# johannes-graeter/limo

Measured on NVIDIA H100. Metric: BA windows/s (30 KF, 3k LM, 40k obs), higher is better.
Workload: dtype f64

## Files before the change

### limo_b200/csrc/kba_api.cu

```cuda
#include <algorithm>
#include <atomic>
#include <chrono>
#include <cmath>
#include <cstdio>
#include <cstdlib>
#include <cstring>
#include <functional>
#include <memory>
#include <string>
#include <thread>
#include <vector>

#include <cuda_runtime.h>

#include "kba_b200.h"
#include "kba_kernels.h"

using namespace kba;

static thread_local std::string g_last_error;
static int fail(int code, const std::string& msg) {
    g_last_error = msg;
    return code;
}
// ... 707 lines not shown
    b->bd.nr_cap_max = p.nr_cap_max; b->bd.fused = p.fused; b->bd.p_split = p.p_split;
    b->bd.solve_tiled = p.solve_tiled; b->bd.solve_split = p.solve_split; b->bd.solve_banded = p.solve_banded;
}

static int batch_create(kba_handle* h, int32_t n_windows, const kba_window* w, const int* rows_of, Purpose purpose, kba_batch** out) {
    if (!h || !w || !out || n_windows <= 0) return fail(KBA_ERR_BAD_ARG, "bad argument to kba_batch_create");
    CU(cudaSetDevice(h->device));
    std::string why;
    for (int i = 0; i < n_windows; ++i) {
        const int rc = validate_window(&w[i], why);
        if (rc != KBA_OK) return fail(rc, "window " + std::to_string(i) + ": " + why);
        if (w[i].n_kf < 3 && !w[i].landmarks_fixed)
            return fail(KBA_ERR_NOT_ENOUGH_KF, "window " + std::to_string(i) + ": fewer than 3 keyframes");
    }
    kba_batch* b = new kba_batch();
    b->h = h;
    BatchDev& bd = b->bd;
    bd.n_win = n_windows;
    b->desc_h.resize(n_windows);
    std::vector<WinShape> shapes(n_windows);
    long long kf = 0, cam = 0, lm = 0, obs = 0, chunks = 0, soff = 0, gp = 0, groups = 0;
    for (int i = 0; i < n_windows; ++i) {
        WinDesc& d = b->desc_h[i];
        memset(&d, 0, sizeof d);
        d.n_kf = w[i].n_kf; d.n_cam = w[i].n_cam; d.n_lm = w[i].n_lm; d.n_obs = w[i].n_obs; d.n_gp = w[i].n_gp;
        d.kf_off = (int)kf; d.cam_off = (int)cam; d.lm_off = (int)lm; d.obs_off = (int)obs; d.gp_off = (int)gp;
        d.chunk_off = (int)chunks; d.n_chunks = (w[i].n_lm + 31) / 32;
        d.grp_off = (int)groups; d.n_groups = (w[i].n_lm + 7) / 8;
        groups += d.n_groups;
        d.scale_kf0 = w[i].scale_kf0; d.scale_kf1 = w[i].scale_kf1;
        d.scale_weight = w[i].scale_weight; d.scale_value = w[i].scale_value;
        WinShape& ws = shapes[i];
        ws.rows = rows_of ? rows_of[i] : reduced_rows(w[i].n_kf, w[i].n_gp > 0 || w[i].plane_reg_weight > 0);
        ws.free_rows = window_rows(w[i]);
        ws.n_chunks = d.n_chunks; ws.n_groups = d.n_groups; ws.n_lm = w[i].n_lm;
        d.nr_cap = nr_cap_of(ws.rows);
        d.plane_reg_weight = w[i].plane_reg_weight; d.plane_dist_fixed = w[i].plane_dist_fixed;
        d.s_off = soff;
        soff += (long long)d.nr_cap * d.nr_cap;
        kf += w[i].n_kf; cam += w[i].n_cam; lm += w[i].n_lm; obs += w[i].n_obs; chunks += d.n_chunks; gp += w[i].n_gp;
        bd.max_obs = std::max(bd.max_obs, w[i].n_obs); bd.max_lm = std::max(bd.max_lm, w[i].n_lm);
        bd.max_kf = std::max(bd.max_kf, w[i].n_kf); bd.max_gp = std::max(bd.max_gp, w[i].n_gp);
    }
    b->lc.knobs = read_knobs();
    b->lc.plan = make_plan(shapes.data(), n_windows, h->sm_count, b->lc.knobs, purpose);
    apply_plan(b);
    const int nr_cap_max = b->lc.plan.nr_cap_max;
    if (obs > 2000000000LL) { b->release(); delete b; return fail(KBA_ERR_CAPACITY, "batch exceeds 2^31 observations"); }
    if (nr_cap_max > kMaxReducedRows) {
        b->release();
        delete b;
        return fail(KBA_ERR_CAPACITY, "reduced system larger than 1344 rows (128 keyframes with ground-plane blocks)");
    }
    bd.tot_kf = kf; bd.tot_cam = cam; bd.tot_lm = lm; bd.tot_obs = obs; bd.tot_chunks = (int)chunks; bd.tot_gp = gp;
    bd.tot_groups = (int)groups;
    b->lc.sm_count = h->sm_count;
    bd.cost_parts = std::max((bd.max_obs + 255) / 256, (bd.max_obs / 16 + bd.max_lm / 32 + 4 + 7) / 8);
    bd.bs_parts = (bd.max_lm + 15) / 16;
    const bool hp = !b->lc.plan.device_pack;
    int bad = 0;
    bad |= b->desc.alloc(n_windows, true);
    bad |= b->pose0.alloc(7 * kf, true); bad |= b->plane0.alloc(4 * kf, true); bad |= b->kf_fixed.alloc(kf, true);
    bad |= b->cam.alloc(kCamStride * cam, true);
    bad |= b->lm0.alloc(3 * lm, hp); bad |= b->lm_weight.alloc(lm, hp); bad |= b->lm_ptr.alloc(lm + n_windows, hp);
    bad |= b->obs_kf.alloc(obs, hp); bad |= b->obs_cam.alloc(obs, hp); bad |= b->obs_lm.alloc(obs, hp);
    bad |= b->obs_u.alloc(obs, hp); bad |= b->obs_v.alloc(obs, hp); bad |= b->obs_d.alloc(obs, hp);
    bad |= b->kf_ptr.alloc(kf + n_windows, hp); bad |= b->pm_lm.alloc(obs, hp); bad |= b->pm_cam.alloc(obs, hp);
    bad |= b->pm_u.alloc(obs, hp); bad |= b->pm_v.alloc(obs, hp); bad |= b->pm_d.alloc(obs, hp);
    bad |= b->chunk_lm0.alloc(chunks, hp); bad |= b->chunk_lm1.alloc(chunks, hp);
    bad |= b->chunk_k0.alloc(chunks, hp); bad |= b->chunk_k1.alloc(chunks, hp);
    bad |= b->lm_orig.alloc(lm, hp); bad |= b->obs_rank.alloc(obs, hp);
    if (hp) bad |= b->obs_orig.alloc(obs, true);
    bad |= b->grp_k0.alloc(groups, hp); bad |= b->grp_k1.alloc(groups, hp);
    if (b->lc.plan.device_pack) {
        bad |= b->r_lm_ptr.alloc(lm + n_windows, true); bad |= b->r_obs_kf.alloc(obs, true); bad |= b->r_obs_cam.alloc(obs, true);
        bad |= b->r_obs_u.alloc(obs, true); bad |= b->r_obs_v.alloc(obs, true); bad |= b->r_obs_d.alloc(obs, true);
        bad |= b->r_lm_pos.alloc(3 * lm, true); bad |= b->r_lm_weight.alloc(lm, true); bad |= b->r_gp_lm.alloc(gp, true);
        bad |= b->lm_user.alloc(3 * lm, true); bad |= b->rej_user.alloc(lm, true);
        bad |= b->dev_alloc(&b->raw.lm_inv, lm);
    }
    bad |= b->dev_alloc(&bd.grp_t0, groups); bad |= b->dev_alloc(&bd.grp_t1, groups); bad |= b->dev_alloc(&bd.grp_rs, groups);
    bad |= b->dev_alloc(&bd.grp_tiles, groups);
    bad |= b->dev_alloc(&bd.lin_tile, (size_t)(obs / 16) + (size_t)(lm / 32) + 4 * (size_t)n_windows + 4);
#ifdef KBA_PROF
    bad |= b->dev_alloc(&bd.prof, 16);
    if (!bad) cudaMemset(bd.prof, 0, 16 * sizeof(unsigned long long));
#endif
    bad |= b->dev_alloc(&bd.rt[0], (size_t)kPoseStride * kf); bad |= b->dev_alloc(&bd.rt[1], (size_t)kPoseStride * kf);
    {
        bd.panel_cap = 0;
        bd.vpanel = nullptr;
        bad |= b->dev_alloc(&bd.chunk_poff, chunks); bad |= b->dev_alloc(&bd.chunk_rs, chunks);
    }
    bad |= b->dev_alloc(&bd.chunk_t0, chunks); bad |= b->dev_alloc(&bd.chunk_t1, chunks); bad |= b->dev_alloc(&bd.obs_row, obs);
    bad |= b->state.alloc(n_windows, true); bad |= b->log.alloc((size_t)n_windows * kIterLogCap, true); bad |= b->wsp.alloc(n_windows, true);
    for (int q = 0; q < 2; ++q) { bad |= b->pose_out[q].alloc(7 * kf, true); bad |= b->lm_out[q].alloc(3 * lm, hp); }
    bad |= b->lm_active.alloc(lm, hp); bad |= b->n_active.alloc(1, true); bad |= b->jac_obs.alloc(1, true);
    bad |= b->plane_out[0].alloc(4 * kf, true); bad |= b->plane_out[1].alloc(4 * kf, true);
    bad |= b->gp_lm.alloc(gp, hp); bad |= b->gp_kf.alloc(gp, true); bad |= b->gp_weight.alloc(gp, true); bad |= b->gp_of_lm.alloc(lm, hp); bad |= b->gp_shared.alloc(gp, hp);
    bad |= b->dev_alloc(&bd.gp_lin, 14 * gp); bad |= b->dev_alloc(&bd.vgp, 30 * gp);
    bad |= b->dev_alloc(&bd.gp_kfb, gp ? 65 * (size_t)kf : 0);
    bad |= b->dev_alloc(&bd.gp_cost_x, n_windows); bad |= b->dev_alloc(&bd.gp_cost_c, n_windows);
    bad |= b->dev_alloc(&bd.off_pose, kf); bad |= b->dev_alloc(&bd.off_dir, kf); bad |= b->dev_alloc(&bd.off_dist, kf);
    bad |= b->dev_alloc(&bd.bkf, 27 * kf);
    bad |= b->dev_alloc(&bd.scale_f, (size_t)n_windows * nr_cap_max); bad |= b->dev_alloc(&bd.lambda_f, (size_t)n_windows * nr_cap_max);
    bad |= b->dev_alloc(&bd.grad_f, (size_t)n_windows * nr_cap_max); bad |= b->dev_alloc(&bd.delta_f, (size_t)n_windows * nr_cap_max);
    bad |= b->dev_alloc(&bd.lm_scale, 3 * lm); bad |= b->dev_alloc(&bd.lm_linv, 6 * lm); bad |= b->dev_alloc(&bd.lm_z, 3 * lm);
    bad |= b->dev_alloc(&bd.lm_g, 3 * lm); bad |= b->dev_alloc(&bd.lm_lambda, 3 * lm); bad |= b->dev_alloc(&bd.trim_val, 3 * lm);
    bad |= b->dev_alloc(&bd.trim_reject, lm);
    bad |= b->dev_alloc(&bd.res, 3 * obs); bad |= b->dev_alloc(&bd.jp, 18 * obs);
    if (!bd.fused) bad |= b->dev_alloc(&bd.jl, 9 * obs);
    else { bad |= b->dev_alloc(&bd.vobs, 18 * obs); bad |= b->dev_alloc(&bd.lm_run, lm); }
    bad |= b->dev_alloc(&bd.cost_part_x, (size_t)n_windows * bd.cost_parts); bad |= b->dev_alloc(&bd.cost_part_c, (size_t)n_windows * bd.cost_parts);
    bad |= b->dev_alloc(&bd.bs_part, (size_t)n_windows * bd.bs_parts * 4);
    bad |= b->dev_alloc(&bd.sred, (size_t)soff * bd.p_split); bad |= b->dev_alloc(&bd.amat, (size_t)soff);
    bad |= b->dev_alloc(&bd.chol_w, (size_t)n_windows * 32 * 32); bad |= b->dev_alloc(&bd.chol_invd, (size_t)n_windows * nr_cap_max);
    if (bad) {
        const std::string msg = std::string("device/pinned allocation failed: ") + cudaGetErrorString(cudaGetLastError());
        b->release(); delete b;
        return fail(KBA_ERR_CUDA, msg);
    }
    bd.desc = b->desc.d; bd.state = b->state.d; bd.log = b->log.d; bd.wsp = b->wsp.d;
    bd.pose0 = b->pose0.d; bd.plane0 = b->plane0.d; bd.pose[0] = b->pose_out[0].d; bd.pose[1] = b->pose_out[1].d;
    bd.kf_fixed = b->kf_fixed.d; bd.cam = b->cam.d;
    bd.lm0 = b->lm0.d; bd.lm[0] = b->lm_out[0].d; bd.lm[1] = b->lm_out[1].d; bd.lm_weight = b->lm_weight.d;
    bd.lm_active = b->lm_active.d; bd.lm_ptr = b->lm_ptr.d;
    bd.obs_kf = b->obs_kf.d; bd.obs_cam = b->obs_cam.d; bd.obs_lm = b->obs_lm.d;
    bd.obs_u = b->obs_u.d; bd.obs_v = b->obs_v.d; bd.obs_d = b->obs_d.d;
    bd.kf_ptr = b->kf_ptr.d; bd.pm_lm = b->pm_lm.d; bd.pm_cam = b->pm_cam.d; bd.pm_u = b->pm_u.d; bd.pm_v = b->pm_v.d; bd.pm_d = b->pm_d.d;
    bd.chunk_lm0 = b->chunk_lm0.d; bd.chunk_lm1 = b->chunk_lm1.d; bd.chunk_k0 = b->chunk_k0.d; bd.chunk_k1 = b->chunk_k1.d;
    bd.lm_orig = b->lm_orig.d;
    bd.obs_rank = b->obs_rank.d;
    bd.grp_k0 = b->grp_k0.d; bd.grp_k1 = b->grp_k1.d;
    bd.plane[0] = b->plane_out[0].d; bd.plane[1] = b->plane_out[1].d;
    bd.gp_lm = b->gp_lm.d; bd.gp_kf = b->gp_kf.d; bd.gp_weight = b->gp_weight.d; bd.gp_of_lm = b->gp_of_lm.d; bd.gp_shared = b->gp_shared.d;
    bd.n_active = b->n_active.d;
    bd.jac_obs = b->jac_obs.d;
    if (b->lc.plan.device_pack) {
        PackRaw& r = b->raw;
        r.lm_ptr = b->r_lm_ptr.d; r.obs_kf = b->r_obs_kf.d; r.obs_cam = b->r_obs_cam.d;
        r.obs_u = b->r_obs_u.d; r.obs_v = b->r_obs_v.d; r.obs_d = b->r_obs_d.d;
        r.lm_pos = b->r_lm_pos.d; r.lm_weight = b->r_lm_weight.d; r.gp_lm = b->r_gp_lm.d; r.obs_orig = nullptr;
    }
    {
        cudaError_t e = cudaMemset(bd.jac_obs, 0, sizeof(unsigned long long));
        if (e == cudaSuccess) e = cudaEventCreate(&b->ev_a);
        if (e == cudaSuccess) e = cudaEventCreate(&b->ev_b);
        if (e == cudaSuccess) e = cudaEventCreateWithFlags(&b->ev_poll, (h->blocking_sync ? cudaEventBlockingSync : 0) | cudaEventDisableTiming);
        if (e == cudaSuccess) e = cudaEventCreateWithFlags(&b->ev_poll2, (h->blocking_sync ? cudaEventBlockingSync : 0) | cudaEventDisableTiming);
        if (e == cudaSuccess && b->loop_pass.alloc(1, true)) e = cudaErrorMemoryAllocation;
        if (e == cudaSuccess) e = configure_kernels(nr_cap_max);
        if (e == cudaSuccess && purpose == Purpose::TrackLarge) e = configure_kernels(kTiledMaxRows);
        if (e == cudaSuccess && b->lc.plan.device_pack) e = configure_pack();
        if (e != cudaSuccess) { b->release(); delete b; return fail(KBA_ERR_CUDA, cudaGetErrorString(e)); }
    }
    *out = b;
    const int rc = batch_upload(b, n_windows, w, rows_of);
    if (rc != KBA_OK) { b->release(); delete b; *out = nullptr; }
    return rc;
}

int kba_batch_create(kba_handle* h, int32_t n_windows, const kba_window* w, kba_batch** out) {
    return batch_create(h, n_windows, w, nullptr, Purpose::Batch, out);
}

int kba_batch_upload(kba_batch* b, int32_t n_windows, const kba_window* w) { return batch_upload(b, n_windows, w, nullptr); }
// ... 3917 lines not shown
```

### limo_b200/csrc/kba_device.cuh

```cuda
#pragma once
#include <cstdint>
#include <cuda_runtime.h>

#include "kba_plan.h"

namespace kba {

constexpr int kMaxCam = 8;
constexpr int kPoseStride = 12;
constexpr int kCamStride = 16;
constexpr int kIterLogCap = 160;

struct WinDesc {
    int n_kf, n_cam, n_lm, n_obs, n_gp;
    int kf_off, cam_off, lm_off, obs_off, gp_off;
    int chunk_off, n_chunks;
    int grp_off, n_groups;
    int scale_kf0, scale_kf1;
    double scale_weight, scale_value;
    double plane_reg_weight;
    int plane_dist_fixed, landmarks_fixed;
    int speed_kf;
    int idle;
    double speed_weight, speed_dt;
    double speed_v_before[3];
    double speed_T_origin_before[7];
    long long s_off;
    int nr_cap;
    int max_rank;
    long long panel_off;
};

enum Phase : int { PH_SOLVE_BEGIN = 0, PH_ITERATE = 1, PH_TRIM = 2, PH_DONE = 3 };

struct SolveSummary {
    double initial_cost, final_cost;
    int num_iterations, num_successful_steps, termination, num_landmarks, num_residual_blocks, pad;
};

struct IterRecord {
    double cost, cost_change, gradient_max_norm, step_norm, relative_decrease, radius;
    int iteration, solve_index, valid, successful;
};

struct WinState {
    int phase;
    int cur;
    int need_linearize;
    int iter0;
    int solve_index;
    int round;
    int rounds_total;
    int retried;
    int is_final;
    int max_iter;
    int iteration;
    int num_invalid;
    int last_successful;
    int n_f;
    int nr;
    int eval_failed;
    int solve_failed;
    int log_n;
    int n_solves;
    int n_lin_tiles;
    double radius, decrease_factor;
    double x_cost, x_norm, gmax;
    double f_model, f_step_sq, f_xnorm_sq, f_gmax;
    unsigned long long t_solve_start;
    SolveSummary solves[8];
};

struct SolveParams;
struct BatchDev {
    int n_win;
    int max_obs, max_lm, max_kf, max_gp;
    long long tot_obs, tot_lm, tot_kf, tot_cam, tot_gp;
    WinDesc* desc;
    WinState* state;
    IterRecord* log;
    double* pose0;
    double* plane0;
    double* pose[2];
    double* rt[2];
    double* plane[2];
    uint8_t* kf_fixed;
    int* off_pose;
    int* off_dir;
    int* off_dist;
    double* bkf;
    double* scale_f;
    double* cam;
    double* lm0;
    double* lm[2];
    double* lm_weight;
    uint8_t* lm_active;
    uint8_t* lm_active0;
    int* lm_ptr;
    double* lm_scale;
    double* lm_linv;
    double* lm_z;
    double* lm_g;
    double* lm_lambda;
    double* trim_val;
    uint8_t* trim_reject;
    int* obs_kf;
    int* obs_cam;
    int* obs_lm;
    int* obs_rank;
    float* obs_u, *obs_v, *obs_d;
    int* kf_ptr;
    int* pm_lm;
    int* pm_cam;
    float* pm_u, *pm_v, *pm_d;
    double* res;
    double* jp;
    double* jl;
    double* vpanel;
    long long panel_cap;
    int* chunk_poff;
    int* chunk_rs;
    double* cost_part_x;
    double* cost_part_c;
    int cost_parts;
    int sharded;
    int lm_begin, lm_total;
    int shard_rank, shard_world;
    double* xs;
    double* x_send;
    double* x_recv;
    double* trim_send;
    double* trim_glob;
    uint8_t* reject_glob;
    int shard_cost_parts;
    int shard_gp;
    double* gp_send;
    double* gp_kf_glob;
    uint8_t* act_glob;
    uint8_t* kf_gp_glob;
    int precision;
    int solve_tiled;
    int solve_split;
    int solve_banded;
    double* chol_w;
    double* chol_invd;
    double* bs_part;
    int bs_parts;
    int nr_cap_max;
    double* sred;
    int p_split;
    double* delta_f;
    double* lambda_f;
    double* grad_f;
    double* amat;
    int* chunk_lm0;
    int* chunk_lm1;
    int* chunk_k0;
    int* chunk_k1;
    int* chunk_t0;
    int* chunk_t1;
    int* obs_row;
    int* lm_orig;
    int tot_chunks;
    int fused;
    int* grp_k0;
    int* grp_k1;
    int* grp_t0;
    int* grp_t1;
    int* grp_tiles;
    int* grp_rs;
    double* vobs;
    int4* lm_run;
    int lin1;
    int2* lin_tile;
    unsigned long long* prof;
    int tot_groups;
    int* n_active;
    unsigned long long* jac_obs;
    int* gp_lm;
    int* gp_kf;
    double* gp_weight;
    int* gp_of_lm;
    int* gp_shared;
    double* gp_lin;
    double* vgp;
    double* gp_kfb;
    double* gp_cost_x;
    double* gp_cost_c;
    const SolveParams* wsp;
};

struct SolveParams {
    double gp_huber, gp_quantile;
    double depth_thres, reprojection_thres, depth_quantile, reprojection_quantile;
    double function_tolerance, gradient_tolerance, parameter_tolerance;
    double initial_radius, max_radius, min_radius, min_relative_decrease, min_lm_diagonal, max_lm_diagonal;
    int trim_solver_iterations, final_solver_iterations, min_residual_groups, max_consecutive_invalid_steps;
    double max_solver_time;
    int rounds_override, min_landmarks_for_trimming, num_rounds_option, pad_;
};

__device__ __forceinline__ unsigned long long global_timer_ns() {
    unsigned long long t;
    asm volatile("mov.u64 %0, %%globaltimer;" : "=l"(t));
    return t;
}

template <typename T>
__host__ __device__ inline void quat_to_rot(const T* q, T* R) {
    const T w = q[0], x = q[1], y = q[2], z = q[3];
    const T tx = 2 * x, ty = 2 * y, tz = 2 * z;
    const T twx = tx * w, twy = ty * w, twz = tz * w, txx = tx * x, txy = ty * x, txz = tz * x;
    const T tyy = ty * y, tyz = tz * y, tzz = tz * z;
    R[0] = 1 - (tyy + tzz); R[1] = txy - twz;       R[2] = txz + twy;
    R[3] = txy + twz;       R[4] = 1 - (txx + tzz); R[5] = tyz - twx;
    R[6] = txz - twy;       R[7] = tyz + twx;       R[8] = 1 - (txx + tyy);
}

__host__ __device__ inline void pose_plus(const double* p, const double* d, double* o) {
    const double nd = sqrt(d[0] * d[0] + d[1] * d[1] + d[2] * d[2]);
    if (nd > 0.0) {
        const double s = sin(nd) / nd, c = cos(nd);
        const double q0 = c, q1 = s * d[0], q2 = s * d[1], q3 = s * d[2];
        o[0] = q0 * p[0] - q1 * p[1] - q2 * p[2] - q3 * p[3];
        o[1] = q0 * p[1] + q1 * p[0] + q2 * p[3] - q3 * p[2];
        o[2] = q0 * p[2] - q1 * p[3] + q2 * p[0] + q3 * p[1];
        o[3] = q0 * p[3] + q1 * p[2] - q2 * p[1] + q3 * p[0];
    } else {
        o[0] = p[0]; o[1] = p[1]; o[2] = p[2]; o[3] = p[3];
    }
    o[4] = p[4] + d[3]; o[5] = p[5] + d[4]; o[6] = p[6] + d[5];
}

template <typename T, bool kCost = true>
__device__ inline void cauchy(T b, T w, T s, T& half_rho, T& sqrt_rho1) {
    const T sum = T(1) + s / b;
    half_rho = kCost ? T(0.5) * w * b * log(sum) : T(0);
    sqrt_rho1 = sqrt(w / sum);
}

template <typename T, bool kM, bool kCost = true>
__device__ __forceinline__ bool eval_factored(const T* __restrict__ pose, const T* __restrict__ cam, const T p[3], T u, T v,
                                              T d, T wt, T b_repr, T b_depth, T r[3], T m[9], T a[3], T& half_rho_sum,
                                              T raw[2]) {
    a[0] = pose[0] * p[0] + pose[1] * p[1] + pose[2] * p[2];
    a[1] = pose[3] * p[0] + pose[4] * p[1] + pose[5] * p[2];
    a[2] = pose[6] * p[0] + pose[7] * p[1] + pose[8] * p[2];
    const T x0 = a[0] + pose[9], x1 = a[1] + pose[10], x2 = a[2] + pose[11];
    const T c0 = cam[0] * x0 + cam[1] * x1 + cam[2] * x2 + cam[9];
    const T c1 = cam[3] * x0 + cam[4] * x1 + cam[5] * x2 + cam[10];
    const T c2 = cam[6] * x0 + cam[7] * x1 + cam[8] * x2 + cam[11];
    if (!(fabs(c2) >= T(0.01))) return false;
    const bool has_d = d > T(0);
    const T rd = has_d ? c2 - d : T(0);
    const T f = cam[12], iz = T(1) / c2;
    const T xn = c0 * iz, yn = c1 * iz;
    const T ru = f * xn + cam[13] - u, rv = f * yn + cam[14] - v;
// ... 196 lines not shown
```

### limo_b200/csrc/kba_kernels.cu

```cuda
#include "kba_device.cuh"
#include "kba_kernels.h"
#include "kba_regularisers.cuh"
#include "kba_controller.cuh"
#include "kba_prep.cuh"
#include "kba_linearize.cuh"

#include <cfloat>
#include <cstdio>
#include <cstdlib>
#include <cmath>
#include <type_traits>

namespace kba {

__global__ void __launch_bounds__(256) k_shard_planes(BatchDev bd) {
    if (bd.state[0].phase != PH_SOLVE_BEGIN) return;
    const WinDesc& wd = bd.desc[0];
    for (int k = threadIdx.x; k < wd.n_kf; k += blockDim.x) bd.kf_gp_glob[k] = 0;
    __syncthreads();
    for (int j = threadIdx.x; j < bd.lm_total; j += blockDim.x) {
        const int kp = (int)bd.gp_kf_glob[j];
        if (kp > 0 && bd.act_glob[j]) bd.kf_gp_glob[kp - 1] = 1;
    }
}

constexpr int kBeginThreads = 1024;
__global__ void __launch_bounds__(kBeginThreads) k_solve_begin(BatchDev bd) {
    const int w = blockIdx.x;
    const SolveParams& sp = bd.wsp[w];
    WinState& st = bd.state[w];
    if (st.phase != PH_SOLVE_BEGIN) return;
    const WinDesc wd = bd.desc[w];
    __shared__ int s_has[kMaxKf];
    __shared__ int s_plane[kMaxKf];
    __shared__ int s_cnt[3];
    __shared__ int s_tile_chunk[513];
    for (int k = threadIdx.x; k < wd.n_kf; k += blockDim.x) { s_has[k] = 0; s_plane[k] = 0; }
    if (threadIdx.x < 3) s_cnt[threadIdx.x] = 0;
    __syncthreads();
    {
        int n_gp_act = 0;
        for (int gi = threadIdx.x; gi < wd.n_gp; gi += blockDim.x) {
            const size_t G = (size_t)wd.gp_off + gi;
            if (!bd.lm_active[wd.lm_off + bd.gp_lm[G]]) continue;
            s_has[bd.gp_kf[G]] = 1;
            s_plane[bd.gp_kf[G]] = 1;
            n_gp_act++;
        }
        atomicAdd(&s_cnt[2], n_gp_act);
    }
    const int* lm_ptr = bd.lm_ptr + wd.lm_off + w;
    int n_lm_in = 0, n_blocks = 0;
    for (int j = threadIdx.x; j < wd.n_lm; j += blockDim.x) {
        if (!bd.lm_active[wd.lm_off + j]) continue;
        const int o0 = lm_ptr[j], o1 = lm_ptr[j + 1];
        if (o1 > o0) n_lm_in++;
        for (int o = o0; o < o1; ++o) {
            s_has[bd.obs_kf[wd.obs_off + o]] = 1;
            n_blocks += (bd.obs_d[wd.obs_off + o] > 0.0f) ? 2 : 1;
        }
    }
    atomicAdd(&s_cnt[0], n_lm_in);
    atomicAdd(&s_cnt[1], n_blocks);
    if (bd.sharded)
        for (int k = threadIdx.x; k < wd.n_kf; k += blockDim.x) {
            s_has[k] = 1;
            if (bd.shard_gp && bd.kf_gp_glob[k]) s_plane[k] = 1;
        }
    __syncthreads();
    if (threadIdx.x == 0) {
        if (wd.scale_weight > 0) { s_has[wd.scale_kf0] = 1; s_has[wd.scale_kf1] = 1; }
        if (wd.speed_weight > 0) s_has[wd.speed_kf] = 1;
        if (wd.landmarks_fixed) s_cnt[0] = 0;
        const bool chain = wd.plane_reg_weight > 0 && wd.n_kf > 1;
        int n = 0, n_reg = 0;
        for (int k = 0; k < wd.n_kf; ++k) {
            const bool fixed = bd.kf_fixed[wd.kf_off + k];
            const bool var = (s_has[k] || chain) && !fixed;
            bd.off_pose[wd.kf_off + k] = var ? n : -1;
            if (var) n += 6;
            const bool pl = (s_plane[k] || chain) && !fixed;
            bd.off_dir[wd.kf_off + k] = pl ? n : -1;
            if (pl) n += 3;
            const bool pd = pl && !wd.plane_dist_fixed;
            bd.off_dist[wd.kf_off + k] = pd ? n : -1;
            if (pd) n += 1;
        }
        if (chain) n_reg = 3 * (wd.n_kf - 1) + wd.n_kf;
        st.n_f = n;
        st.nr = (n + 1 + 7) & ~7;
        st.radius = sp.initial_radius;
        st.decrease_factor = 2.0;
        st.iteration = 0;
        st.num_invalid = 0;
        st.last_successful = 0;
        st.need_linearize = 1;
        st.iter0 = 1;
        st.eval_failed = 0;
        st.solve_failed = 0;
        st.max_iter = st.is_final ? sp.final_solver_iterations
                                  : (st.retried ? 3 * sp.trim_solver_iterations : sp.trim_solver_iterations);
        SolveSummary& s = st.solves[st.solve_index];
        s.initial_cost = s.final_cost = 0.0;
        s.num_iterations = 0; s.num_successful_steps = 0; s.termination = 1;
        s.num_landmarks = s_cnt[0];
        s.num_residual_blocks = s_cnt[1] + s_cnt[2] + n_reg + (wd.scale_weight > 0 ? 1 : 0) + (wd.speed_weight > 0 ? 1 : 0);
        st.t_solve_start = global_timer_ns();
        st.phase = PH_ITERATE;
    }
    __syncthreads();
    for (int o = threadIdx.x; o < wd.n_obs; o += blockDim.x) {
        const size_t oo = (size_t)wd.obs_off + o;
        const bool act = bd.lm_active[wd.lm_off + bd.obs_lm[oo]];
        bd.obs_row[oo] = act ? bd.off_pose[wd.kf_off + bd.obs_kf[oo]] : -1;
    }
    for (int c = threadIdx.x; c < (bd.fused ? 0 : wd.n_chunks); c += blockDim.x) {
        int r0 = 1 << 30, r1 = -1;
        for (int k = bd.chunk_k0[wd.chunk_off + c]; k <= bd.chunk_k1[wd.chunk_off + c]; ++k) {
            const int off = bd.off_pose[wd.kf_off + k], od = bd.off_dir[wd.kf_off + k], oz = bd.off_dist[wd.kf_off + k];
// ... 2076 lines not shown
```

### limo_b200/csrc/kba_linearize.cuh

```cuda
#pragma once
#include <type_traits>
#include "kba_device.cuh"

namespace kba {

constexpr int kLinThreads = 256;
constexpr int kLinWarps = kLinThreads / 32;

__host__ __device__ __forceinline__ int lin_tile_bound(int n_obs, int n_lm) { return n_obs / 16 + n_lm / 32 + 4; }
__device__ __forceinline__ size_t lin_tile_offset(const WinDesc& wd, int w) {
    return (size_t)(wd.obs_off / 16) + (size_t)(wd.lm_off / 32) + 4 * (size_t)w;
}

__device__ inline void build_lin_tiles(const BatchDev& bd, const WinDesc& wd, WinState& st, int w, int* s_chunk ) {
    const int* lm_ptr = bd.lm_ptr + wd.lm_off + w;
    int2* tiles = bd.lin_tile + lin_tile_offset(wd, w);
    const int per = max(64, (wd.n_lm + 511) / 512);
    const int n_chunks = (wd.n_lm + per - 1) / per;
    for (int pass = 0; pass < 2; ++pass) {
        for (int c = threadIdx.x; c < n_chunks; c += blockDim.x) {
            const int j0 = c * per, j1 = min(wd.n_lm, j0 + per);
            int n = 0, t_start = 0, t_cnt = 0;
            int2* out = tiles + (pass ? s_chunk[c] : 0);
            int o0 = lm_ptr[j0];
            for (int j = j0; j < j1; ++j) {
                const int o1 = lm_ptr[j + 1], k = o1 - o0;
                if (k > 0) {
                    const bool over = k > 32;
                    if (t_cnt > 0 && (over || t_cnt + k > 32)) { if (pass) out[n] = make_int2(t_start, t_cnt); ++n; t_cnt = 0; }
                    if (!over) { if (t_cnt == 0) t_start = o0; t_cnt += k; }
                }
                o0 = o1;
            }
            if (t_cnt > 0) { if (pass) out[n] = make_int2(t_start, t_cnt); ++n; }
            if (!pass) s_chunk[c] = n;
        }
        __syncthreads();
        if (!pass) {
            if (threadIdx.x == 0) {
                int acc = 0;
                for (int c = 0; c < n_chunks; ++c) { const int t = s_chunk[c]; s_chunk[c] = acc; acc += t; }
                if (acc > lin_tile_bound(wd.n_obs, wd.n_lm)) acc = 0;
                st.n_lin_tiles = acc;
                s_chunk[512] = acc;
            }
            __syncthreads();
            if (s_chunk[512] == 0) return;
        }
    }
}

constexpr int kLinMinBlocks = 3;
constexpr size_t kLinStaticSmem = sizeof(double) * (kFusedMaxKf * kPoseStride + kMaxCam * kCamStride + kLinWarps * 9 * 33 +
                                                    kLinWarps * 32 * 9 + kLinWarps + 4) +
                                  sizeof(int) * (kLinWarps * 6 * 32 + kLinWarps) + sizeof(uint64_t);
static_assert(kLinStaticSmem <= 48 * 1024, "k_linearize: static shared memory over 48 KB");
template <bool kLoop>
__global__ void __launch_bounds__(kLinThreads, kLinMinBlocks) k_linearize(BatchDev bd, int n_units) {
    const int w = blockIdx.y;
    WinState& st = bd.state[w];
    if (st.phase != PH_ITERATE) return;
    const WinDesc& wd = bd.desc[w];
    const volatile WinState& vst = st;
    const auto n_tiles = [&] { return vst.n_lin_tiles; };
    const auto lin = [&] { return vst.need_linearize != 0; };
    const auto want_cost = [&] { return vst.need_linearize != 0 && vst.iter0 != 0; };
    if (wd.landmarks_fixed && !want_cost()) return;
    const int tid = threadIdx.x, lane = tid & 31, warp = tid >> 5;
    __shared__ __align__(16) double s_pose[kFusedMaxKf * kPoseStride];
    __shared__ __align__(16) double s_cam[kMaxCam * kCamStride];
    __shared__ __align__(8) uint64_t s_bar;
    __shared__ double s_cg[kLinWarps][9][33];
    __shared__ double s_ma[kLinWarps][32][9];
    __shared__ int s_ix[kLinWarps][6][32];
    __shared__ double s_red[kLinWarps];
    __shared__ int s_cnt[kLinWarps];
    __shared__ double s_prm[4];
    for (int unit = blockIdx.x; unit < n_units; unit += gridDim.x) {
    asm volatile("" ::: "memory");
    if (unit * kLinWarps >= n_tiles()) {
        if (tid == 0 && want_cost()) bd.cost_part_x[(size_t)w * bd.cost_parts + unit] = 0.0;
        if constexpr (!kLoop) return;
        continue;
    }
    const size_t base = (size_t)wd.obs_off;
    const int* lm_ptr = bd.lm_ptr + wd.lm_off + w;
    const int t = unit * kLinWarps + warp;
    int2 tile = make_int2(0, 0);
    if (t < n_tiles()) tile = bd.lin_tile[lin_tile_offset(wd, w) + t];
    const bool have = lane < tile.y;
    const int o = tile.x + lane;
    int j = 0, kf = 0, cam = 0, row0 = -1, p0 = 0, p1 = 0;
    float mu = 0.f, mv = 0.f, md = 0.f;
    double p[3] = {0, 0, 0}, wgt = 0.0;
    bool act = false;
    if (have) {
        const size_t oo = base + o;
        j = bd.obs_lm[oo];
        kf = bd.obs_kf[oo]; cam = bd.obs_cam[oo]; row0 = bd.obs_row[oo];
        mu = bd.obs_u[oo]; mv = bd.obs_v[oo]; md = bd.obs_d[oo];
        p0 = lm_ptr[j]; p1 = lm_ptr[j + 1];
        act = bd.lm_active[wd.lm_off + j] != 0;
        const double* lmp = bd.lm[st.cur] + 3 * (size_t)(wd.lm_off + j);
        p[0] = lmp[0]; p[1] = lmp[1]; p[2] = lmp[2];
        wgt = bd.lm_weight[wd.lm_off + j];
    }
    int (*six)[32] = s_ix[warp];
    if (unit == (int)blockIdx.x) {
        if (tid == 0) {
            const SolveParams& sp = bd.wsp[w];
            s_prm[0] = sp.reprojection_thres * sp.reprojection_thres; s_prm[1] = sp.depth_thres * sp.depth_thres;
            s_prm[2] = sp.min_lm_diagonal; s_prm[3] = sp.max_lm_diagonal;
        }
        stage_window_bulk(wd, bd.rt[st.cur], bd.cam, s_pose, s_cam, &s_bar);
    }
    six[0][lane] = kf; six[1][lane] = row0; six[2][lane] = wd.obs_off + p0; six[3][lane] = p1 - p0; six[4][lane] = wd.lm_off + j;
    six[5][lane] = have ? 1 | (act ? 2 : 0) | ((p0 - tile.x) << 2) : 0;
    double* sma = s_ma[warp][lane];
    bool ok = false;
    double hr = 0.0;
    double cg[9] = {0, 0, 0, 0, 0, 0, 0, 0, 0};
    if (act) {
        const auto evaluate = [&](auto with_cost) {
            double r[3], m[9], raw[2];
            const double br = s_prm[0], bdp = s_prm[1];
            ok = eval_factored<double, true, decltype(with_cost)::value>(s_pose + kPoseStride * kf, s_cam + kCamStride * cam, p,
                                                                          (double)mu, (double)mv, (double)md, wgt, br, bdp, r, m,
                                                                          sma + 6, hr, raw);
            if (!ok) return;
            {
                unsigned t;
                asm volatile("mov.u32 %0, %%tid.x;" : "=r"(t));
                s_ix[t >> 5][5][t & 31] |= 128;
            }
            gram_factored(m, sma);
            const double* R = s_pose + kPoseStride * reinterpret_cast<volatile int*>(six[0])[lane];
            double jl[9];
#pragma unroll
            for (int i = 0; i < 3; ++i) {
#pragma unroll
                for (int c = 0; c < 3; ++c) jl[3 * i + c] = m[3 * i] * R[c] + m[3 * i + 1] * R[3 + c] + m[3 * i + 2] * R[6 + c];
            }
            cg[0] = jl[0] * jl[0] + jl[3] * jl[3] + jl[6] * jl[6];
            cg[1] = jl[0] * jl[1] + jl[3] * jl[4] + jl[6] * jl[7];
            cg[2] = jl[0] * jl[2] + jl[3] * jl[5] + jl[6] * jl[8];
            cg[3] = jl[1] * jl[1] + jl[4] * jl[4] + jl[7] * jl[7];
            cg[4] = jl[1] * jl[2] + jl[4] * jl[5] + jl[7] * jl[8];
            cg[5] = jl[2] * jl[2] + jl[5] * jl[5] + jl[8] * jl[8];
#pragma unroll
            for (int c = 0; c < 3; ++c) cg[6 + c] = jl[c] * r[0] + jl[3 + c] * r[1] + jl[6 + c] * r[2];
        };
        if (want_cost()) evaluate(std::true_type{});
        else evaluate(std::false_type{});
        if (!ok) {
            hr = 0.0;
            if (lin()) st.eval_failed = 1;
        }
    }
    {
        const double cs = warp_sum(hr);
        const int dn = __reduce_add_sync(0xffffffffu, ok ? 1 : 0);
        if (lane == 0) { s_red[warp] = cs; s_cnt[warp] = dn; }
    }
    if (!wd.landmarks_fixed) {
        double (*sw)[33] = s_cg[warp];
#pragma unroll
        for (int q = 0; q < 9; ++q) sw[q][lane] = cg[q];
        __syncwarp();
        const int L = six[4][lane];
        const bool in_tile = six[5][lane] & 1, active = six[5][lane] & 2;
        const int seg0 = (six[5][lane] >> 2) & 31;
        const int klen = six[3][lane];
        double tt_ld[3] = {0.0, 0.0, 0.0};
        if (active && !st.iter0) {
#pragma unroll
            for (int e = 0; e < 3; ++e) tt_ld[e] = bd.lm_scale[3 * (size_t)L + e];
        }
        if (in_tile) {
            for (int q = lane - seg0; q < 9; q += klen) {
                double sacc = 0.0;
                for (int l = seg0; l < seg0 + klen; ++l) sacc += sw[q][l];
                sw[q][seg0] = sacc;
            }
        }
        __syncwarp();
        if (active) {
            double c[6], g[3];
#pragma unroll
            for (int q = 0; q < 6; ++q) c[q] = sw[q][seg0];
#pragma unroll
            for (int q = 0; q < 3; ++q) g[q] = sw[6 + q][seg0];
            const bool first = lane == seg0;
            const int gl = (wd.n_gp > 0) ? bd.gp_of_lm[L] : -1;
            const size_t TG = (size_t)bd.tot_gp, G = (size_t)wd.gp_off + (gl >= 0 ? gl : 0);
            double gjl[3] = {0, 0, 0};
            if (gl >= 0) {
                gjl[0] = bd.gp_lin[11 * TG + G]; gjl[1] = bd.gp_lin[12 * TG + G]; gjl[2] = bd.gp_lin[13 * TG + G];
                const double gr = bd.gp_lin[G];
                c[0] += gjl[0] * gjl[0]; c[1] += gjl[0] * gjl[1]; c[2] += gjl[0] * gjl[2];
                c[3] += gjl[1] * gjl[1]; c[4] += gjl[1] * gjl[2]; c[5] += gjl[2] * gjl[2];
// ... 86 lines not shown
```

Measured before the change: 1454.

## Bin-pack active landmark observations into warp tiles for non-cost linearize passes

Adds a second tiling scheme that packs only active landmarks' observations into 32-lane warp tiles with a first-fit-decreasing bin packing over strided landmark subsets, stored as per-lane observation indices. The linearize kernel uses packed tiles when no cost evaluation is needed and keeps consecutive tiles for the cost pass. The aim is to reduce idle lanes and skip inactive landmarks, at the cost of extra tile build work, a 32x larger per-lane index buffer, and an extra global load per lane.

```diff
diff --git a/limo_b200/csrc/kba_api.cu b/limo_b200/csrc/kba_api.cu
--- a/limo_b200/csrc/kba_api.cu
+++ b/limo_b200/csrc/kba_api.cu
@@ -813,6 +813,7 @@
     bad |= b->dev_alloc(&bd.grp_t0, groups); bad |= b->dev_alloc(&bd.grp_t1, groups); bad |= b->dev_alloc(&bd.grp_rs, groups);
     bad |= b->dev_alloc(&bd.grp_tiles, groups);
     bad |= b->dev_alloc(&bd.lin_tile, (size_t)(obs / 16) + (size_t)(lm / 32) + 4 * (size_t)n_windows + 4);
+    bad |= b->dev_alloc(&bd.lin_ptile, 32 * ((size_t)(obs / 16) + (size_t)(lm / 32) + 4 * (size_t)n_windows + 4));
 #ifdef KBA_PROF
     bad |= b->dev_alloc(&bd.prof, 16);
     if (!bad) cudaMemset(bd.prof, 0, 16 * sizeof(unsigned long long));
diff --git a/limo_b200/csrc/kba_device.cuh b/limo_b200/csrc/kba_device.cuh
--- a/limo_b200/csrc/kba_device.cuh
+++ b/limo_b200/csrc/kba_device.cuh
@@ -64,6 +64,7 @@
     int log_n;
     int n_solves;
     int n_lin_tiles;
+    int n_lin_ptiles;
     double radius, decrease_factor;
     double x_cost, x_norm, gmax;
     double f_model, f_step_sq, f_xnorm_sq, f_gmax;
@@ -173,6 +174,7 @@
     int4* lm_run;
     int lin1;
     int2* lin_tile;
+    int* lin_ptile;
     unsigned long long* prof;
     int tot_groups;
     int* n_active;
diff --git a/limo_b200/csrc/kba_kernels.cu b/limo_b200/csrc/kba_kernels.cu
--- a/limo_b200/csrc/kba_kernels.cu
+++ b/limo_b200/csrc/kba_kernels.cu
@@ -34,7 +34,7 @@
     __shared__ int s_has[kMaxKf];
     __shared__ int s_plane[kMaxKf];
     __shared__ int s_cnt[3];
-    __shared__ int s_tile_chunk[513];
+    __shared__ int s_tile_chunk[2 * (kLinMaxChunks + 1)];
     for (int k = threadIdx.x; k < wd.n_kf; k += blockDim.x) { s_has[k] = 0; s_plane[k] = 0; }
     if (threadIdx.x < 3) s_cnt[threadIdx.x] = 0;
     __syncthreads();
diff --git a/limo_b200/csrc/kba_linearize.cuh b/limo_b200/csrc/kba_linearize.cuh
--- a/limo_b200/csrc/kba_linearize.cuh
+++ b/limo_b200/csrc/kba_linearize.cuh
@@ -1,39 +1,44 @@
 #pragma once
 #include <type_traits>
 #include "kba_device.cuh"
+#include "kba_lintile.h"
 
 namespace kba {
 
 constexpr int kLinThreads = 256;
 constexpr int kLinWarps = kLinThreads / 32;
 
-__host__ __device__ __forceinline__ int lin_tile_bound(int n_obs, int n_lm) { return n_obs / 16 + n_lm / 32 + 4; }
 __device__ __forceinline__ size_t lin_tile_offset(const WinDesc& wd, int w) {
     return (size_t)(wd.obs_off / 16) + (size_t)(wd.lm_off / 32) + 4 * (size_t)w;
 }
 
-__device__ inline void build_lin_tiles(const BatchDev& bd, const WinDesc& wd, WinState& st, int w, int* s_chunk ) {
+__device__ inline void build_lin_tiles(const BatchDev& bd, const WinDesc& wd, WinState& st, int w,
+                                       int* s_chunk ) {
     const int* lm_ptr = bd.lm_ptr + wd.lm_off + w;
+    const uint8_t* lm_active = bd.lm_active + wd.lm_off;
     int2* tiles = bd.lin_tile + lin_tile_offset(wd, w);
-    const int per = max(64, (wd.n_lm + 511) / 512);
+    int* ptiles = bd.lin_ptile + 32 * lin_tile_offset(wd, w);
+    int* s_pchunk = s_chunk + kLinMaxChunks + 1;
+    const int per = max(kLinChunkMin, (wd.n_lm + kLinMaxChunks - 1) / kLinMaxChunks);
     const int n_chunks = (wd.n_lm + per - 1) / per;
+    const int n_pc = lin_pack_chunks(wd.n_lm);
+    const int pper = (n_pc + kLinMaxChunks - 1) / kLinMaxChunks;
+    const int n_pg = pper > 0 ? (n_pc + pper - 1) / pper : 0;
+    const int worker = (threadIdx.x & 31) * (blockDim.x >> 5) + (threadIdx.x >> 5);
+    const auto active = [&](int j) { return lm_active[j] != 0; };
     for (int pass = 0; pass < 2; ++pass) {
         for (int c = threadIdx.x; c < n_chunks; c += blockDim.x) {
-            const int j0 = c * per, j1 = min(wd.n_lm, j0 + per);
-            int n = 0, t_start = 0, t_cnt = 0;
             int2* out = tiles + (pass ? s_chunk[c] : 0);
-            int o0 = lm_ptr[j0];
-            for (int j = j0; j < j1; ++j) {
-                const int o1 = lm_ptr[j + 1], k = o1 - o0;
-                if (k > 0) {
-                    const bool over = k > 32;
-                    if (t_cnt > 0 && (over || t_cnt + k > 32)) { if (pass) out[n] = make_int2(t_start, t_cnt); ++n; t_cnt = 0; }
-                    if (!over) { if (t_cnt == 0) t_start = o0; t_cnt += k; }
-                }
-                o0 = o1;
-            }
-            if (t_cnt > 0) { if (pass) out[n] = make_int2(t_start, t_cnt); ++n; }
+            const int n = lin_tiles_consecutive(lm_ptr, c * per, min(wd.n_lm, (c + 1) * per), [&](int i, int first, int cnt) {
+                if (pass) out[i] = make_int2(first, cnt);
+            });
             if (!pass) s_chunk[c] = n;
+        }
+        for (int g = worker; g < n_pg; g += blockDim.x) {
+            int n = 0;
+            for (int c = g * pper; c < min(n_pc, (g + 1) * pper); ++c)
+                n += lin_tiles_packed(lm_ptr, wd.n_lm, c, n_pc, active, pass ? ptiles + 32 * (size_t)(s_pchunk[g] + n) : nullptr);
+            if (!pass) s_pchunk[g] = n;
         }
         __syncthreads();
         if (!pass) {
@@ -41,11 +46,19 @@
                 int acc = 0;
                 for (int c = 0; c < n_chunks; ++c) { const int t = s_chunk[c]; s_chunk[c] = acc; acc += t; }
                 if (acc > lin_tile_bound(wd.n_obs, wd.n_lm)) acc = 0;
-                st.n_lin_tiles = acc;
-                s_chunk[512] = acc;
+                s_chunk[kLinMaxChunks] = acc;
+            } else if (threadIdx.x == 32) {
+                int acc = 0;
+                for (int g = 0; g < n_pg; ++g) { const int t = s_pchunk[g]; s_pchunk[g] = acc; acc += t; }
+                s_pchunk[kLinMaxChunks] = acc;
             }
             __syncthreads();
-            if (s_chunk[512] == 0) return;
+            const bool none = s_chunk[kLinMaxChunks] == 0;
+            if (threadIdx.x == 0) {
+                st.n_lin_tiles = s_chunk[kLinMaxChunks];
+                st.n_lin_ptiles = none ? 0 : s_pchunk[kLinMaxChunks];
+            }
+            if (none) return;
         }
     }
 }
@@ -62,7 +75,6 @@
     if (st.phase != PH_ITERATE) return;
     const WinDesc& wd = bd.desc[w];
     const volatile WinState& vst = st;
-    const auto n_tiles = [&] { return vst.n_lin_tiles; };
     const auto lin = [&] { return vst.need_linearize != 0; };
     const auto want_cost = [&] { return vst.need_linearize != 0 && vst.iter0 != 0; };
     if (wd.landmarks_fixed && !want_cost()) return;
@@ -78,18 +90,25 @@
     __shared__ double s_prm[4];
     for (int unit = blockIdx.x; unit < n_units; unit += gridDim.x) {
     asm volatile("" ::: "memory");
-    if (unit * kLinWarps >= n_tiles()) {
-        if (tid == 0 && want_cost()) bd.cost_part_x[(size_t)w * bd.cost_parts + unit] = 0.0;
+    const int v_lin = vst.need_linearize, v_iter0 = vst.iter0, v_cons = vst.n_lin_tiles, v_pack = vst.n_lin_ptiles;
+    const bool cost_pass = (v_lin != 0) & (v_iter0 != 0);
+    const int n_tiles = cost_pass ? v_cons : v_pack;
+    if (unit * kLinWarps >= n_tiles) {
+        if (tid == 0 && cost_pass) bd.cost_part_x[(size_t)w * bd.cost_parts + unit] = 0.0;
         if constexpr (!kLoop) return;
         continue;
     }
     const size_t base = (size_t)wd.obs_off;
     const int* lm_ptr = bd.lm_ptr + wd.lm_off + w;
     const int t = unit * kLinWarps + warp;
-    int2 tile = make_int2(0, 0);
-    if (t < n_tiles()) tile = bd.lin_tile[lin_tile_offset(wd, w) + t];
-    const bool have = lane < tile.y;
-    const int o = tile.x + lane;
+    int o = -1;
+    if (t < n_tiles) {
+        const size_t slot = lin_tile_offset(wd, w) + t;
+        const int2 tile = bd.lin_tile[slot];
+        const int po = bd.lin_ptile[32 * slot + lane];
+        o = cost_pass ? (lane < tile.y ? tile.x + lane : -1) : po;
+    }
+    const bool have = o >= 0;
     int j = 0, kf = 0, cam = 0, row0 = -1, p0 = 0, p1 = 0;
     float mu = 0.f, mv = 0.f, md = 0.f;
     double p[3] = {0, 0, 0}, wgt = 0.0;
@@ -115,7 +134,7 @@
         stage_window_bulk(wd, bd.rt[st.cur], bd.cam, s_pose, s_cam, &s_bar);
     }
     six[0][lane] = kf; six[1][lane] = row0; six[2][lane] = wd.obs_off + p0; six[3][lane] = p1 - p0; six[4][lane] = wd.lm_off + j;
-    six[5][lane] = have ? 1 | (act ? 2 : 0) | ((p0 - tile.x) << 2) : 0;
+    six[5][lane] = have ? 1 | (act ? 2 : 0) | ((lane - (o - p0)) << 2) : 0;
     double* sma = s_ma[warp][lane];
     bool ok = false;
     double hr = 0.0;
diff --git a/limo_b200/csrc/kba_lintile.h b/limo_b200/csrc/kba_lintile.h
--- /dev/null
+++ b/limo_b200/csrc/kba_lintile.h
@@ -0,0 +1,68 @@
+#pragma once
+
+#if defined(__CUDACC__)
+#define KBA_HD __host__ __device__
+#else
+#define KBA_HD
+#endif
+
+namespace kba {
+
+constexpr int kLinChunkMin = 64;
+constexpr int kLinPackChunk = 128;
+constexpr int kLinMaxChunks = 512;
+
+KBA_HD inline int lin_tile_bound(int n_obs, int n_lm) { return n_obs / 16 + n_lm / 32 + 4; }
+
+template <class Emit>
+KBA_HD inline int lin_tiles_consecutive(const int* lm_ptr, int j0, int j1, Emit emit) {
+    int n = 0, t_start = 0, t_cnt = 0;
+    int o0 = lm_ptr[j0];
+    for (int j = j0; j < j1; ++j) {
+        const int o1 = lm_ptr[j + 1], k = o1 - o0;
+        if (k > 0) {
+            const bool over = k > 32;
+            if (t_cnt > 0 && (over || t_cnt + k > 32)) { emit(n++, t_start, t_cnt); t_cnt = 0; }
+            if (!over) { if (t_cnt == 0) t_start = o0; t_cnt += k; }
+        }
+        o0 = o1;
+    }
+    if (t_cnt > 0) emit(n++, t_start, t_cnt);
+    return n;
+}
+
+KBA_HD inline int lin_pack_chunks(int n_lm) { return (n_lm + kLinPackChunk - 1) / kLinPackChunk; }
+
+template <class Active>
+KBA_HD inline int lin_tiles_packed(const int* lm_ptr, int n_lm, int c, int n_chunks, Active active, int* out) {
+    constexpr unsigned char kNone = 0xff;
+    unsigned char head[33], next[kLinPackChunk], room[kLinPackChunk];
+    for (int k = 0; k <= 32; ++k) head[k] = kNone;
+    for (int i = (n_lm - 1 - c) / n_chunks; i >= 0; --i) {
+        const int j = c + i * n_chunks;
+        const int k = lm_ptr[j + 1] - lm_ptr[j];
+        if (k < 1 || k > 32 || !active(j)) continue;
+        next[i] = head[k];
+        head[k] = (unsigned char)i;
+    }
+    int n = 0;
+    for (int k = 32; k >= 1; --k) {
+        int t = 0;
+        for (int i = head[k]; i != kNone; i = next[i]) {
+            while (t < n && room[t] < k) ++t;
+            if (t == n) room[n++] = 32;
+            const int l0 = 32 - room[t];
+            room[t] = (unsigned char)(room[t] - k);
+            if (out) {
+                const int o0 = lm_ptr[c + i * n_chunks];
+                for (int q = 0; q < k; ++q) out[32 * t + l0 + q] = o0 + q;
+            }
+        }
+    }
+    if (out)
+        for (int t = 0; t < n; ++t)
+            for (int l = 32 - room[t]; l < 32; ++l) out[32 * t + l] = -1;
+    return n;
+}
+
+}
```

After: 1472, median of 6. 1.3% higher.
